# zxhuang1698/ShapeClipper

Hardware: AMD Instinct MI355X
Metric: train-step images/sec (Pix3D cfg, bs32/GPU) (higher is better)
Workload: dtype f32 (bf16x3-split MFMA, fp32 accumulate)

## Files before the change

### shapeclipper_amd/csrc/block.hip

```cpp
#include <hip/hip_runtime.h>
#include <stdint.h>

#include "shapeclipper_hip.h"


extern "C" int sc_basic_block_forward(const sc_block_args* a, void* stream) {
    if (!a || a->batch <= 0 || a->channels <= 0) return (int)hipErrorInvalidValue;
    const int B = a->batch, C = a->channels, hw = a->hw, HW = hw * hw, G = a->groups;
    auto conv = a->split ? sc_conv3x3_forward_split : sc_conv3x3_forward;
    int rc = conv(a->x, a->pf1, a->y1, a->conv_ws, B, C, C, hw, stream);
    if (rc) return rc;
    rc = sc_bn_act_forward(a->y1, nullptr, a->g1, a->b1, a->a1, a->st1, a->st1 + (size_t)G * C, a->rm1, a->rv1, a->nt1, a->bn_ws, B, C, HW, 1,
                           a->training, G, a->eps1, a->mom1, stream);
    if (rc) return rc;
    rc = conv(a->a1, a->pf2, a->y2, a->conv_ws, B, C, C, hw, stream);
    if (rc) return rc;
    return sc_bn_act_forward(a->y2, a->x, a->g2, a->b2, a->out, a->st2, a->st2 + (size_t)G * C, a->rm2, a->rv2, a->nt2, a->bn_ws, B, C, HW, 1,
                             a->training, G, a->eps2, a->mom2, stream);
}

extern "C" int sc_basic_block_backward(const sc_block_args* a, void* stream) {
    if (!a || a->batch <= 0 || a->channels <= 0 || !a->d_out) return (int)hipErrorInvalidValue;
    const int B = a->batch, C = a->channels, hw = a->hw, HW = hw * hw, G = a->groups;
    auto conv = a->split ? sc_conv3x3_forward_split : sc_conv3x3_forward;
    auto wgrad = a->split ? sc_conv3x3_wgrad_split : sc_conv3x3_wgrad;
    int rc = sc_bn_act_backward(a->d_out, a->y2, a->out, a->g2, a->b2, a->st2, a->st2 + (size_t)G * C, a->bn_ws, a->dy2, a->need_dx ? a->dres : nullptr,
                                a->dgb2, a->dgb2 + C, B, C, HW, 1, a->training, G, stream);
    if (rc) return rc;
    rc = conv(a->dy2, a->pb2, a->da1, a->conv_ws, B, C, C, hw, stream);
    if (rc) return rc;
    if (a->gw2) {
        rc = wgrad(a->dy2, a->a1, a->gw2, a->wgrad_ws, B, C, C, hw, stream);
        if (rc) return rc;
    }
    rc = sc_bn_act_backward(a->da1, a->y1, nullptr, a->g1, a->b1, a->st1, a->st1 + (size_t)G * C, a->bn_ws, a->dy1, nullptr, a->dgb1, a->dgb1 + C, B,
                            C, HW, 1, a->training, G, stream);
    if (rc) return rc;
    if (a->need_dx) {
        rc = sc_conv3x3_forward_add(a->dy1, a->pb1, a->dres, a->dx, a->conv_ws, B, C, C, hw, a->split, stream);
        if (rc) return rc;
    }
    if (a->gw1) rc = wgrad(a->dy1, a->x, a->gw1, a->wgrad_ws, B, C, C, hw, stream);
    return rc;
}
```

### shapeclipper_amd/csrc/conv3x3.hip

```cpp
#include <hip/hip_runtime.h>

#include <map>
#include <mutex>
#include <tuple>
#include <vector>

#include "grid_cus.hpp"
#include "shapeclipper_hip.h"

#ifndef SC_CONV_SPANS
#define SC_CONV_SPANS 1
#endif
#ifndef SC_CONV_ABLATE
#define SC_CONV_ABLATE 0
#endif

namespace sc {

#ifdef SC_CONV_PROFILE
__device__ unsigned long long* conv_prof_buf = nullptr;
#define CV_STAMP(ID) { const unsigned long long t_ = __builtin_amdgcn_s_memrealtime(); if (conv_prof_buf && tid == 0) conv_prof_buf[(size_t)g * 32 + (ID)] = t_; }
#else
#define CV_STAMP(ID)
#endif

typedef float f32x16 __attribute__((ext_vector_type(16)));
typedef __bf16 cv_bf16x8 __attribute__((ext_vector_type(8)));
typedef __bf16 cv_bf16x2 __attribute__((ext_vector_type(2)));
typedef __attribute__((address_space(3))) void* lptr_cv_t;

__device__ __forceinline__ void conv_glds16(const void* gsrc, unsigned lds_dst) {
// ... 395 lines not shown
        } else {
            float4* dst = reinterpret_cast<float4*>(partial + ((size_t)g * 2 + (item - sp.rounds)) * C::TILE);
#pragma unroll
            for (int i = 0; i < WM; ++i)
#pragma unroll
                for (int j = 0; j < WN; ++j)
#pragma unroll
                    for (int q = 0; q < 4; ++q) {
                        const float4 v = make_float4(acc[i][j][4 * q], acc[i][j][4 * q + 1], acc[i][j][4 * q + 2], acc[i][j][4 * q + 3]);
                        float4* d = dst + (((wave * WM + i) * WN + j) * 4 + q) * 64 + lane;
                        *d = v;
                    }
        }
#ifdef SC_CONV_PROFILE
        asm volatile("s_waitcnt vmcnt(0)" ::: "memory");
        CV_STAMP(sid + 3)
        if (conv_prof_buf && tid == 0) conv_prof_buf[(size_t)g * 32 + sid + 4] = (unsigned long long)(kb1 - kb0);
#endif
    }
    CV_STAMP(25)
}

template <class C>
__global__ __launch_bounds__(C::NT) void conv3x3_fixup_kernel(const float* __restrict__ partial, float* __restrict__ out, int batch,
                                                              int cin, int cout, int G, const int* __restrict__ spans,
                                                              const float* __restrict__ addend) {
    const int tid = threadIdx.x, lane = tid & 63, wave = tid >> 6;
    const int wm = wave / C::WGN, wn = wave % C::WGN;
    const int npix = batch * C::HWO, nct = (cout + C::CT - 1) / C::CT, tiles = ((npix + C::PT - 1) / C::PT) * nct * (C::BD2 ? 4 : 1);
    const int nk = conv_nk<C>(cin);
    const ConvSplit sp = conv_split(tiles, nk, G);
#ifdef SC_CONV_PROFILE
    if (conv_prof_buf && tid == 0) conv_prof_buf[(size_t)(8192 + blockIdx.x * 4 + blockIdx.y) * 2] = __builtin_amdgcn_s_memrealtime();
#endif
    const int t = blockIdx.x, r0 = 4 * blockIdx.y;
    const long long u0 = (long long)t * nk, u1 = u0 + nk;
    const int g_first = conv_span_owner(spans, sp, u0, G), g_last = conv_span_owner(spans, sp, u1 - 1, G);
    if (g_first == g_last && conv_span_at(spans, sp, g_first, nk) == u0 && conv_span_at(spans, sp, g_first + 1, nk) == u1) return;
    float acc[C::WM][C::WN][4];
#pragma unroll
    for (int i = 0; i < C::WM; ++i)
#pragma unroll
        for (int j = 0; j < C::WN; ++j)
#pragma unroll
            for (int r = 0; r < 4; ++r) acc[i][j][r] = 0.f;
    for (int g = g_first; g <= g_last; ++g) {
        const int which = (int)(conv_span_at(spans, sp, g, nk) / nk) == t ? 0 : 1;
        const float4* src = reinterpret_cast<const float4*>(partial + ((size_t)g * 2 + which) * C::TILE);
#pragma unroll
        for (int i = 0; i < C::WM; ++i)
#pragma unroll
            for (int j = 0; j < C::WN; ++j) {
                const float4 v = src[(((wave * C::WM + i) * C::WN + j) * 4 + (r0 >> 2)) * 64 + lane];
                acc[i][j][0] += v.x; acc[i][j][1] += v.y; acc[i][j][2] += v.z; acc[i][j][3] += v.w;
            }
    }
    const int tile = sp.rounds * G + t;
    int phase, pt, ct;
    conv_tile_decode<C>(tile, nct, phase, pt, ct);
#pragma unroll
    for (int j = 0; j < C::WN; ++j) {
        const int p = pt * C::PT + (wn * C::WN + j) * 32 + (lane & 31);
        if (p >= npix) continue;
        int cs;
        float* ob = conv_out_pixel<C>(out, p, phase, cout, cs);
#pragma unroll
        for (int i = 0; i < C::WM; ++i)
#pragma unroll
            for (int r = 0; r < 4; ++r) {
                const int co = ct * C::CT + (wm * C::WM + i) * 32 + r + 2 * r0 + 4 * (lane >> 5);
                if (co < cout) ob[(size_t)co * cs] = addend ? acc[i][j][r] + addend[(ob - out) + (size_t)co * cs] : acc[i][j][r];
            }
    }
#ifdef SC_CONV_PROFILE
    asm volatile("s_waitcnt vmcnt(0)" ::: "memory");
    if (conv_prof_buf && tid == 0) conv_prof_buf[(size_t)(8192 + blockIdx.x * 4 + blockIdx.y) * 2 + 1] = __builtin_amdgcn_s_memrealtime();
#endif
}

__device__ __forceinline__ float conv_w_at(const float* __restrict__ w, int cin, int cout, int co, int ci, int tap, int transpose_flip) {
    return transpose_flip ? w[((size_t)ci * cout + co) * 9 + (8 - tap)] : w[((size_t)co * cin + ci) * 9 + tap];
}
__device__ __forceinline__ unsigned conv_bf16_piece(float v, int pc) {
    const __bf16 h0 = (__bf16)v;
    const float r1 = v - (float)h0;
    const __bf16 h1 = (__bf16)r1;
    const __bf16 h2 = (__bf16)(r1 - (float)h1);
    const __bf16 h = pc == 0 ? h0 : pc == 1 ? h1 : h2;
    return (unsigned)__builtin_bit_cast(unsigned short, h);
}
__device__ __forceinline__ float conv_pack_word(const float* __restrict__ w, unsigned t, int CT, int nk, int cin, int cout, int flip,
                                                bool split) {
    if (!split) {
        const int s4 = (int)(t & 3);
        t >>= 2;
        const int cl = (int)(t % CT);
        t /= CT;
        const int h = (int)(t & 1);
        t >>= 1;
        const int tap = (int)(t % 9);
// ... 193 lines not shown
        U[G] = total;
        return pos >= total;
    };
    int lo = 2 * ((total + G - 1) / G), hi = lo + 4 * ov2 + 4;
    while (!build(hi)) hi += 2 * nk;
    while (lo < hi) {
        const int mid = (lo + hi) / 2;
        if (build(mid)) hi = mid; else lo = mid + 1;
    }
    (void)build(hi);
    SpanTable& t = cache[key];
    t.host = U;
    if (hipMalloc(&t.dev, (size_t)(G + 1) * sizeof(int)) != hipSuccess ||
        hipMemcpyAsync(t.dev, t.host.data(), (size_t)(G + 1) * sizeof(int), hipMemcpyHostToDevice, st) != hipSuccess ||
        hipStreamSynchronize(st) != hipSuccess) {
        (void)hipGetLastError();
        if (t.dev) (void)hipFree(t.dev);
        t.dev = nullptr;
    }
    return t.dev;
}

template <class C>
static int launch_conv(const float* x, const float* wpack, float* out, float* workspace, int batch, int cin, int cout, hipStream_t st,
                       const float* addend = nullptr) {
    if (cin % C::CB || batch <= 0) return (int)hipErrorInvalidValue;
    const int tiles = ((batch * C::HWO + C::PT - 1) / C::PT) * ((cout + C::CT - 1) / C::CT) * (C::BD2 ? 4 : 1), nk = conv_nk<C>(cin);
    const int G = conv_grid() * C::WGS_PER_CU;
    if (C::SPLIT && (long long)batch * cin * C::HW * 4 > 0x7fffffffLL) return (int)hipErrorInvalidValue;
    (void)hipFuncSetAttribute((const void*)conv3x3_kernel<C>, hipFuncAttributeMaxDynamicSharedMemorySize, C::LDS_BYTES);
    const ConvSplit sp = conv_split(tiles, nk, G);
    const int* spans = (SC_CONV_SPANS && sp.tail_tiles > 0 && sp.per_wg <= nk) ? conv_spans(sp.tail_tiles, nk, G, C::PT >= 512 ? 2 : 3, st) : nullptr;
    hipLaunchKernelGGL((conv3x3_kernel<C>), dim3(G), dim3(C::NT), C::LDS_BYTES, st, x, wpack, out, workspace, batch, cin, cout, spans, addend);
    if (sp.tail_tiles > 0)
        hipLaunchKernelGGL((conv3x3_fixup_kernel<C>), dim3(sp.tail_tiles, 4), dim3(C::NT), 0, st, workspace, out, batch, cin, cout, G, spans, addend);
    return (int)hipGetLastError();
}

}

extern "C" int sc_conv3x3_release_tables(void) {
    std::lock_guard<std::mutex> lock(sc::span_mu);
    int dev0 = 0;
    (void)hipGetDevice(&dev0);
    for (auto& kv : sc::span_cache)
        if (kv.second.dev) {
            (void)hipSetDevice(std::get<0>(kv.first));
            (void)hipFree(kv.second.dev);
        }
    sc::span_cache.clear();
    (void)hipSetDevice(dev0);
    return 0;
}

#define SC_CONV_DISPATCH(hw, CALL)                   \
    switch (hw) {                                    \
        case 56: return CALL(sc::Conv56);            \
        case 28: return CALL(sc::Conv28);            \
// ... 144 lines not shown
    }
    if (transpose_flip & 2) {
#define CALL(C) sc::launch_pack<C>(w, w_pack, cin, cout, transpose_flip & 1, (hipStream_t)stream)
        SC_CONV_DISPATCH_SPLIT(hw, CALL)
#undef CALL
    }
#define CALL(C) sc::launch_pack<C>(w, w_pack, cin, cout, transpose_flip & 1, (hipStream_t)stream)
    SC_CONV_DISPATCH(hw, CALL)
#undef CALL
}

extern "C" int sc_conv3x3_forward_add(const float* x, const float* w_pack, const float* addend, float* out, float* workspace, int batch, int cin,
                                      int cout, int hw, int split, void* stream) {
    if (split) {
#define CALL(C) sc::launch_conv<C>(x, w_pack, out, workspace, batch, cin, cout, (hipStream_t)stream, addend)
        SC_CONV_DISPATCH_SPLIT(hw, CALL)
#undef CALL
    }
#define CALL(C) sc::launch_conv<C>(x, w_pack, out, workspace, batch, cin, cout, (hipStream_t)stream, addend)
    SC_CONV_DISPATCH(hw, CALL)
#undef CALL
}

extern "C" int sc_conv3x3_forward(const float* x, const float* w_pack, float* out, float* workspace, int batch, int cin, int cout, int hw,
                                  void* stream) {
#define CALL(C) sc::launch_conv<C>(x, w_pack, out, workspace, batch, cin, cout, (hipStream_t)stream)
    SC_CONV_DISPATCH(hw, CALL)
#undef CALL
}
```

### shapeclipper_amd/csrc/conv3x3_wgrad.hip

```cpp
#include <hip/hip_runtime.h>

#include "grid_cus.hpp"
#include "shapeclipper_hip.h"

namespace sc {

typedef float wg_f32x16 __attribute__((ext_vector_type(16)));

#ifdef SC_WGRAD_PROFILE
__device__ unsigned long long* wgrad_prof_buf = nullptr;
#define WG_STAMP(ID) { const unsigned long long t_ = __builtin_amdgcn_s_memrealtime(); if (wgrad_prof_buf && tid == 0) wgrad_prof_buf[(size_t)blockIdx.x * 16 + (ID)] = t_; }
#define WG_ACCUM(ID, T0) { const unsigned long long t_ = __builtin_amdgcn_s_memrealtime(); if (wgrad_prof_buf && tid == 0) wgrad_prof_buf[(size_t)blockIdx.x * 16 + (ID)] += t_ - (T0); }
#else
#define WG_STAMP(ID)
#endif

template <int W_, int NR_, int NIMG_, int GS_, int S_ = 1>
struct WgCfg {
    static constexpr int W = W_, H = W_, NR = NR_, NIMG = NIMG_, GS = GS_, S = S_;
    static constexpr int HW = W * W;
    static constexpr int XW = S * W, XH = S * H, XHW = XW * XH;
    static constexpr int Wp = S == 1 ? W + 2 : XW + 1;
    static constexpr bool WHOLE = NR == H;
    static constexpr int SLOTW = (W + 2 * GS - 1) / (2 * GS) * (2 * GS);
    static constexpr int ROWS = NIMG * NR;
    static constexpr int NSLOT = ROWS * SLOTW;
    static constexpr int GST = NSLOT + (((NSLOT / GS) & 1) ? 0 : GS);
    static constexpr int PR = S == 1 ? NR + 2 : 2 * NR + 1;
    static constexpr int PATCH = NIMG * PR * Wp;
    static constexpr int LQ = (S == 1 ? PATCH : PATCH + 2 * GS + 2) | 1;
    static constexpr int LDS_FLOATS = 64 * GST + 64 * LQ > 4 * 48 * 64 ? 64 * GST + 64 * LQ : 4 * 48 * 64;
    static constexpr int CHUNK = W == 7 ? 49 : 56;
    static constexpr int RPC = CHUNK / W;
    static constexpr int XCHUNK = XW == 7 ? 49 : 56, XRPC = XCHUNK / XW;
    static constexpr int XROWS = WHOLE ? XH : PR;
    static constexpr int XCH = (XROWS + XRPC - 1) / XRPC, GCH = (NR + RPC - 1) / RPC;
    static constexpr int HR = ROWS / 2;
    static constexpr int GPR = SLOTW / (2 * GS);
    static constexpr int KH_A = HR * SLOTW;
    static constexpr int KH_B = NIMG == 2 ? PR * Wp : S * HR * Wp;
    static constexpr int NBV = S == 1 ? GS + 2 : 2 * GS + 1;
    static_assert(ROWS % 2 == 0 && H % NR == 0 && SLOTW % (2 * GS) == 0 && CHUNK % W == 0 && XCHUNK % XW == 0 && (S == 1 || S == 2), "K-step shape");
    static_assert(LDS_FLOATS * 4 <= 160 * 1024 && 4 * 48 * 64 <= LDS_FLOATS, "LDS");
};

template <class C>
__global__ __launch_bounds__(512, 1) void conv3x3_wgrad_kernel(const float* __restrict__ gy, const float* __restrict__ x,
                                                               float* __restrict__ partial, int batch, int cin, int cout, int S) {
    constexpr int W = C::W, H = C::H, HW = C::HW, Wp = C::Wp, GS = C::GS, NIMG = C::NIMG, NR = C::NR, ST = C::S;
    constexpr int XW = C::XW, XH = C::XH, XHW = C::XHW;
    extern __shared__ float4 wg_smem[];
    float* As = reinterpret_cast<float*>(wg_smem);
    float* Xs = As + 64 * C::GST;
    const int tid = threadIdx.x, lane = tid & 63, wave = __builtin_amdgcn_readfirstlane(tid >> 6), half = lane >> 5;
    const int wt = wave & 3, kh = wave >> 2;
    const int nti = cin / 64;
    const int blk = blockIdx.x / S, s = blockIdx.x - blk * S;
    const int co0 = (blk / nti) * 64, ci0 = (blk % nti) * 64;
    const int nimg_steps = NIMG == 2 ? (batch + 1) / 2 : batch * (H / NR);
    const int k_lo = (int)((long long)s * nimg_steps / S), k_hi = (int)((long long)(s + 1) * nimg_steps / S);

    for (int i = tid; i < C::LDS_FLOATS; i += 512) As[i] = 0.f;

    const bool lane_on = lane < C::CHUNK, xlane_on = lane < C::XCHUNK;
    const int lrow = lane / W, lx = lane - lrow * W;
    const int xlrow = lane / XW, xlx = lane - xlrow * XW;
    float xv[8][C::XCH * NIMG], gv[8][C::GCH * NIMG];
    auto load = [&](int kstep) {
        int b, y0;
        if (NIMG == 2) { b = 2 * kstep; y0 = 0; } else { b = kstep / (H / NR); y0 = (kstep - b * (H / NR)) * NR; }
#pragma unroll
        for (int im = 0; im < NIMG; ++im) {
            const bool img_ok = b + im < batch;
            const float* xb = x + ((size_t)(b + im) * cin + ci0 + 8 * wave) * XHW;
            const float* gb = gy + ((size_t)(b + im) * cout + co0 + 8 * wave) * HW;
#pragma unroll
            for (int c = 0; c < C::XCH; ++c) {
                const int yr = (C::WHOLE ? 0 : ST * y0 - 1) + c * C::XRPC + xlrow;
                const bool ok = xlane_on && img_ok && (unsigned)yr < (unsigned)XH && c * C::XRPC + xlrow < C::XROWS;
                const int off = yr * XW + xlx;
// ... 75 lines not shown
        }
        __syncthreads();
    }

    float* R = As;
#pragma unroll
    for (int pass = 0; pass < 3; ++pass) {
        if (kh == 1) {
#pragma unroll
            for (int t = 0; t < 3; ++t)
#pragma unroll
                for (int r = 0; r < 16; ++r) R[((wt * 3 + t) * 16 + r) * 64 + lane] = acc[pass * 3 + t][r];
        }
        __syncthreads();
        if (kh == 0) {
#pragma unroll
            for (int t = 0; t < 3; ++t)
#pragma unroll
                for (int r = 0; r < 16; ++r) acc[pass * 3 + t][r] += R[((wt * 3 + t) * 16 + r) * 64 + lane];
        }
        __syncthreads();
    }
    if (kh == 0) {
        float* dst = partial + (size_t)blockIdx.x * (64 * 64 * 9);
#pragma unroll
        for (int t = 0; t < 9; ++t)
#pragma unroll
            for (int r = 0; r < 16; ++r) dst[((wt * 9 + t) * 16 + r) * 64 + lane] = acc[t][r];
    }
}

__global__ __launch_bounds__(256) void conv3x3_wgrad_reduce_kernel(const float* __restrict__ partial, float* __restrict__ dw, int cin,
                                                                  int cout, int S) {
    __shared__ float part[4][64];
    const int nti = cin / 64, lane = threadIdx.x & 63, w = threadIdx.x >> 6;
    const int blk = blockIdx.x / 576, e = (blockIdx.x - blk * 576) * 64 + lane;
    const float* src = partial + (size_t)blk * S * 36864 + e;
    float s0 = 0.f, s1 = 0.f;
    int s = w;
    for (; s + 4 < S; s += 8) {
        s0 += src[(size_t)s * 36864];
        s1 += src[(size_t)(s + 4) * 36864];
    }
    if (s < S) s0 += src[(size_t)s * 36864];
    part[w][lane] = s0 + s1;
    __syncthreads();
    if (w == 0) {
        const float sum = (part[0][lane] + part[1][lane]) + (part[2][lane] + part[3][lane]);
        const int r = (e >> 6) & 15, t = (e >> 10) % 9, wt = e / (9 * 1024);
        const int co = (blk / nti) * 64 + (wt >> 1) * 32 + (r & 3) + 8 * (r >> 2) + 4 * (lane >> 5);
        const int ci = (blk % nti) * 64 + (wt & 1) * 32 + (lane & 31);
        dw[((size_t)co * cin + ci) * 9 + t] = sum;
    }
}

using Wg56 = WgCfg<56, 2, 1, 4>;
using Wg28 = WgCfg<28, 4, 1, 2>;
using Wg14 = WgCfg<14, 14, 1, 1>;
using Wg7 = WgCfg<7, 7, 2, 1>;
using Wg28S2 = WgCfg<28, 2, 1, 2, 2>;
using Wg14S2 = WgCfg<14, 2, 1, 1, 2>;
using Wg7S2 = WgCfg<7, 7, 2, 1, 2>;

typedef __bf16 wg_bf16x8 __attribute__((ext_vector_type(8)));
typedef float wg_f32x4 __attribute__((ext_vector_type(4)));
#ifndef SC_WGRAD_S16
#define SC_WGRAD_S16 0
#endif

template <int W_, int NR_, int NIMG_>
struct WsCfg {
    static constexpr int W = W_, H = W_, NR = NR_, NIMG = NIMG_, HW = W * W;
    static constexpr int SLOTS = W == 7 ? 8 : (W + 15) / 16 * 16;
    static constexpr int ROWS = NIMG * NR, NSLOT = ROWS * SLOTS, G = NSLOT / 16;
    static constexpr int ASTR = NSLOT + 8;
    static constexpr int Wp = SLOTS + 2, PR = NR + 2, PATCH = NIMG * PR * Wp;
    static constexpr int BSTR = (PATCH + 3) / 4 * 4 + 2;
    static constexpr bool WHOLE = NR == H;
    static constexpr int LDS_BYTES = 3 * 64 * (ASTR + BSTR) * 2;
    static constexpr int CHUNK = W == 7 ? 49 : 56, RPC = CHUNK / W;
    static constexpr int XROWS = WHOLE ? H : PR;
    static constexpr int XCH = (XROWS + RPC - 1) / RPC, GCH = (NR + RPC - 1) / RPC;
    static_assert(NSLOT % 16 == 0 && H % NR == 0 && LDS_BYTES <= 160 * 1024 && (W >= 14 || (NIMG == 2 && NR == 7)), "K-step shape");
    static constexpr int boff(int g, int h) {
        if (W == 7) { const int r = 2 * g + h; return ((r / 7) * PR + r % 7) * Wp; }
        const int r = g / (SLOTS / 16), gx = g % (SLOTS / 16);
        return ((r / NR) * PR + r % NR) * Wp + 16 * gx + 8 * h;
    }
};

template <class C>
__global__ __launch_bounds__(768, 1) void conv3x3_wgrad_split_kernel(const float* __restrict__ gy, const float* __restrict__ x,
                                                                     float* __restrict__ partial, int batch, int cin, int cout, int S) {
    constexpr int W = C::W, H = C::H, HW = C::HW, Wp = C::Wp, NIMG = C::NIMG, NR = C::NR;
    extern __shared__ float4 wg_smem[];
    __bf16* As = reinterpret_cast<__bf16*>(wg_smem);
    __bf16* Xs = As + 3 * 64 * C::ASTR;
    const int tid = threadIdx.x, lane = tid & 63, wave = __builtin_amdgcn_readfirstlane(tid >> 6), half = lane >> 5;
    const int wt = wave & 3, ky = wave >> 2;
    const int nti = cin / 64;
    const int blk = blockIdx.x / S, s = blockIdx.x - blk * S;
    const int co0 = (blk / nti) * 64, ci0 = (blk % nti) * 64;
    const int nimg_steps = NIMG == 2 ? (batch + 1) / 2 : batch * (H / NR);
    const int k_lo = (int)((long long)s * nimg_steps / S), k_hi = (int)((long long)(s + 1) * nimg_steps / S);

    for (int i = tid; i < C::LDS_BYTES / 16; i += 768) wg_smem[i] = make_float4(0.f, 0.f, 0.f, 0.f);

    const bool lane_on = lane < C::CHUNK, xrole = wave < 8;
    const int lrow = lane / W, lx = lane - lrow * W;
    constexpr int NSV = 8 * C::XCH * NIMG > 16 * C::GCH * NIMG ? 8 * C::XCH * NIMG : 16 * C::GCH * NIMG;
    float sv[NSV];
    auto load = [&](int kstep) {
        int b, y0;
        if (NIMG == 2) { b = 2 * kstep; y0 = 0; } else { b = kstep / (H / NR); y0 = (kstep - b * (H / NR)) * NR; }
        if (xrole) {
#pragma unroll
            for (int im = 0; im < NIMG; ++im) {
                const float* xb = x + ((size_t)(b + im) * cin + ci0 + 8 * wave) * HW;
#pragma unroll
                for (int c = 0; c < C::XCH; ++c) {
                    const int rr = c * C::RPC + lrow, yr = (C::WHOLE ? 0 : y0 - 1) + rr;
                    const bool ok = lane_on && b + im < batch && (unsigned)yr < (unsigned)H && rr < C::XROWS;
                    const int off = yr * W + lx;
#pragma unroll
// ... 143 lines not shown
#pragma unroll
                for (int q = 0; q < 5; ++q) d[pc][q] = Bb[pc * 32 * C::BSTR + bo + q];
            }
#pragma unroll
            for (int term = 0; term < 6; ++term) {
                constexpr int PA[6] = {0, 2, 1, 0, 1, 0}, PB[6] = {2, 0, 1, 1, 0, 0};
                const unsigned* q = d[PB[term]];
                const wg_bf16x8 av = __builtin_bit_cast(wg_bf16x8, a[PA[term]]);
                uint4 b0 = {q[0], q[1], q[2], q[3]}, b2 = {q[1], q[2], q[3], q[4]};
                uint4 b1 = {__builtin_amdgcn_alignbit(q[1], q[0], 16), __builtin_amdgcn_alignbit(q[2], q[1], 16),
                            __builtin_amdgcn_alignbit(q[3], q[2], 16), __builtin_amdgcn_alignbit(q[4], q[3], 16)};
                acc[0] = __builtin_amdgcn_mfma_f32_32x32x16_bf16(av, __builtin_bit_cast(wg_bf16x8, b0), acc[0], 0, 0, 0);
                acc[1] = __builtin_amdgcn_mfma_f32_32x32x16_bf16(av, __builtin_bit_cast(wg_bf16x8, b1), acc[1], 0, 0, 0);
                acc[2] = __builtin_amdgcn_mfma_f32_32x32x16_bf16(av, __builtin_bit_cast(wg_bf16x8, b2), acc[2], 0, 0, 0);
            }
        }
#endif
        __syncthreads();
#ifdef SC_WGRAD_PROFILE
        WG_ACCUM(5, ts1)
#endif
    }
    WG_STAMP(2)
    float* dst = partial + (size_t)blockIdx.x * (64 * 64 * 9);
#if SC_WGRAD_S16
#pragma unroll
    for (int t = 0; t < 3; ++t)
#pragma unroll
        for (int sa = 0; sa < 2; ++sa)
#pragma unroll
            for (int sb = 0; sb < 2; ++sb)
#pragma unroll
                for (int r = 0; r < 4; ++r)
                    dst[((wt * 9 + ky * 3 + t) * 16 + r + 4 * (2 * sa + (q4 >> 1))) * 64 + 16 * sb + l16 + 32 * (q4 & 1)] = acc[t][sa][sb][r];
#else
#pragma unroll
    for (int t = 0; t < 3; ++t)
#pragma unroll
        for (int r = 0; r < 16; ++r) dst[((wt * 9 + ky * 3 + t) * 16 + r) * 64 + lane] = acc[t][r];
#endif
#ifdef SC_WGRAD_PROFILE
    asm volatile("s_waitcnt vmcnt(0)" ::: "memory");
    WG_STAMP(3)
    if (wgrad_prof_buf && tid == 0) wgrad_prof_buf[(size_t)blockIdx.x * 16 + 6] = (unsigned long long)(k_hi - k_lo);
#endif
}

using Ws56 = WsCfg<56, 2, 1>;
using Ws28 = WsCfg<28, 4, 1>;
using Ws14 = WsCfg<14, 7, 1>;
using Ws7 = WsCfg<7, 7, 2>;

static int wg_cus() { return grid_cus(); }
static int wg_splits(int cin, int cout) {
    const int nblk = (cin / 64) * (cout / 64), s = wg_cus() / nblk;
    return s > 0 ? s : 1;
}

template <class C>
static int launch_wgrad(const float* gy, const float* x, float* dw, float* workspace, int batch, int cin, int cout, hipStream_t st) {
    if (cin % 64 || cout % 64 || batch <= 0) return (int)hipErrorInvalidValue;
    const int nblk = (cin / 64) * (cout / 64), S = wg_splits(cin, cout);
    (void)hipFuncSetAttribute((const void*)conv3x3_wgrad_kernel<C>, hipFuncAttributeMaxDynamicSharedMemorySize, C::LDS_FLOATS * 4);
    hipLaunchKernelGGL((conv3x3_wgrad_kernel<C>), dim3(nblk * S), dim3(512), C::LDS_FLOATS * 4, st, gy, x, workspace, batch, cin, cout, S);
    hipLaunchKernelGGL(conv3x3_wgrad_reduce_kernel, dim3(nblk * 576), dim3(256), 0, st, workspace, dw, cin, cout, S);
    return (int)hipGetLastError();
}

template <class C>
static int launch_wgrad_split(const float* gy, const float* x, float* dw, float* workspace, int batch, int cin, int cout, hipStream_t st) {
    if (cin % 64 || cout % 64 || batch <= 0) return (int)hipErrorInvalidValue;
    const int nblk = (cin / 64) * (cout / 64), S = wg_splits(cin, cout);
    (void)hipFuncSetAttribute((const void*)conv3x3_wgrad_split_kernel<C>, hipFuncAttributeMaxDynamicSharedMemorySize, C::LDS_BYTES);
    hipLaunchKernelGGL((conv3x3_wgrad_split_kernel<C>), dim3(nblk * S), dim3(768), C::LDS_BYTES, st, gy, x, workspace, batch, cin, cout, S);
    hipLaunchKernelGGL(conv3x3_wgrad_reduce_kernel, dim3(nblk * 576), dim3(256), 0, st, workspace, dw, cin, cout, S);
    return (int)hipGetLastError();
}

}

#ifdef SC_WGRAD_PROFILE
extern "C" int sc_wgrad_debug_set_prof(unsigned long long* buf) {
    return (int)hipMemcpyToSymbol(HIP_SYMBOL(sc::wgrad_prof_buf), &buf, sizeof(buf));
}
#endif
extern "C" int sc_conv3x3_wgrad_split(const float* gy, const float* x, float* dw, float* workspace, int batch, int cin, int cout, int hw, void* stream) {
    switch (hw) {
        case 56: return sc::launch_wgrad_split<sc::Ws56>(gy, x, dw, workspace, batch, cin, cout, (hipStream_t)stream);
        case 28: return sc::launch_wgrad_split<sc::Ws28>(gy, x, dw, workspace, batch, cin, cout, (hipStream_t)stream);
        case 14: return sc::launch_wgrad_split<sc::Ws14>(gy, x, dw, workspace, batch, cin, cout, (hipStream_t)stream);
        case 7: return sc::launch_wgrad_split<sc::Ws7>(gy, x, dw, workspace, batch, cin, cout, (hipStream_t)stream);
        default: return -1;
    }
}

extern "C" long long sc_conv3x3_wgrad_workspace_floats(int cin, int cout) {
    if (cin <= 0 || cout <= 0 || cin % 64 || cout % 64) return -1;
    return (long long)(cin / 64) * (cout / 64) * sc::wg_splits(cin, cout) * 36864;
}
// ... 20 lines not shown
```

### shapeclipper_amd/ops.py

```python
from __future__ import annotations

import collections
import ctypes
import weakref

import torch

from . import _lib
from .packing import n_tiles

_SCRATCH = {}


def _scratch(tag, dev, n_floats):
    if dev.type != "cuda":
        raise RuntimeError(_lib.NO_CPU)
    key = (tag, dev.index, torch._C._cuda_getCurrentRawStream(dev.index))
    buf = _SCRATCH.get(key)
    if buf is None or buf.numel() < n_floats:
        buf = _SCRATCH[key] = torch.empty(n_floats, device=dev, dtype=torch.float32)
    return buf


SDF_SCRATCH_FLOATS = 256 * 8 * 5 * 1024
# ... 979 lines not shown
def conv3x3_backward_weight(gy, x, split=False):
    lib = _lib.load()
    gy, x = _aligned(gy), _aligned(x)
    B, cout, H, _ = gy.shape
    cin = x.shape[1]
    n = lib.sc_conv3x3_wgrad_workspace_floats(cin, cout)
    if n < 0 or H not in CONV3X3_SIDES or x.shape[0] != B or tuple(x.shape[2:]) != (H, H):
        raise RuntimeError("shapeclipper_amd: sc_conv3x3_wgrad does not take gy %s with x %s" % (tuple(gy.shape), tuple(x.shape)))
    ws = _scratch("conv wgrad", x.device, n)
    dw = torch.empty(cout, cin, 3, 3, device=x.device, dtype=torch.float32)
    fn = lib.sc_conv3x3_wgrad_split if split else lib.sc_conv3x3_wgrad
    _lib.check(fn(_lib.ptr(gy), _lib.ptr(x), _lib.ptr(dw), _lib.ptr(ws), B, cin, cout, H, _lib.stream()), "sc_conv3x3_wgrad")
    return dw


class BlockArgs(ctypes.Structure):
    _fields_ = ([(n, ctypes.c_void_p) for n in ("x", "pf1", "pf2", "pb1", "pb2", "g1", "b1", "g2", "b2", "rm1", "rv1", "rm2", "rv2", "nt1", "nt2",
                                   "y1", "a1", "y2", "out", "st1", "st2", "conv_ws", "bn_ws", "wgrad_ws", "d_out",
                                   "dy2", "dres", "da1", "dy1", "dx", "gw1", "gw2", "dgb1", "dgb2")]
                + [(n, ctypes.c_int) for n in ("batch", "channels", "hw", "groups", "training", "split", "need_dx")]
                + [(n, ctypes.c_float) for n in ("mom1", "eps1", "mom2", "eps2")])


def _wgrad_workspace(x, cin, cout):
    return _scratch("conv wgrad", x.device, _lib.load().sc_conv3x3_wgrad_workspace_floats(cin, cout))


def basic_block_forward(x, pf1, pf2, g1, b1, g2, b2, bn1_state, bn2_state, split, groups):
    B, C, H, _ = x.shape
    rm1, rv1, nt1, training, mom1, eps1 = bn1_state
    rm2, rv2, nt2, _, mom2, eps2 = bn2_state
    y1, a1, y2, out = (torch.empty_like(x) for _ in range(4))
    st = torch.empty(2, 2, groups, C, device=x.device, dtype=torch.float32)
    a = BlockArgs()
    a.x, a.pf1, a.pf2 = x.data_ptr(), pf1.data_ptr(), pf2.data_ptr()
    a.g1, a.b1, a.g2, a.b2 = g1.data_ptr(), b1.data_ptr(), g2.data_ptr(), b2.data_ptr()
    a.rm1, a.rv1, a.nt1, a.rm2, a.rv2, a.nt2 = _p(rm1), _p(rv1), _p(nt1), _p(rm2), _p(rv2), _p(nt2)
    a.y1, a.a1, a.y2, a.out = y1.data_ptr(), a1.data_ptr(), y2.data_ptr(), out.data_ptr()
    a.st1, a.st2 = st[0].data_ptr(), st[1].data_ptr()
    a.conv_ws, a.bn_ws = _conv_workspace(x.device, H, split).data_ptr(), _bn_partial(x, groups)
    a.batch, a.channels, a.hw, a.groups, a.training, a.split = B, C, H, groups, 1 if training else 0, 1 if split else 0
    a.mom1, a.eps1, a.mom2, a.eps2 = mom1, eps1, mom2, eps2
    code = _lib.load().sc_basic_block_forward(ctypes.byref(a), _lib.raw_stream(x.get_device()))
    if code:
        _lib.check(code, "sc_basic_block_forward")
    return out, (y1, a1, y2, st[0], st[1])


def basic_block_backward(d_out, x, saved, out, pb1, pb2, g1, b1, g2, b2, training, split, groups, need_dx, need_w1, need_w2):
    y1, a1, y2, st1, st2 = saved
    B, C, H, _ = x.shape
    dy2, da1, dy1 = (torch.empty_like(x) for _ in range(3))
    dx, dres = (torch.empty_like(x), torch.empty_like(x)) if need_dx else (None, None)
    gw1 = torch.empty(C, C, 3, 3, device=x.device, dtype=torch.float32) if need_w1 else None
    gw2 = torch.empty(C, C, 3, 3, device=x.device, dtype=torch.float32) if need_w2 else None
    dgb = torch.empty(2, 2, C, device=x.device, dtype=torch.float32)
    a = BlockArgs()
    a.x, a.pb1, a.pb2, a.d_out = x.data_ptr(), pb1.data_ptr(), pb2.data_ptr(), d_out.data_ptr()
    a.g1, a.b1, a.g2, a.b2 = g1.data_ptr(), b1.data_ptr(), g2.data_ptr(), b2.data_ptr()
    a.y1, a.a1, a.y2, a.out, a.st1, a.st2 = y1.data_ptr(), a1.data_ptr(), y2.data_ptr(), out.data_ptr(), st1.data_ptr(), st2.data_ptr()
    a.dy2, a.da1, a.dy1, a.dres, a.dx = dy2.data_ptr(), da1.data_ptr(), dy1.data_ptr(), _p(dres), _p(dx)
    a.gw1, a.gw2, a.dgb1, a.dgb2 = _p(gw1), _p(gw2), dgb[0].data_ptr(), dgb[1].data_ptr()
    a.conv_ws, a.bn_ws = _conv_workspace(x.device, H, split).data_ptr(), _bn_partial(x, groups)
    a.wgrad_ws = _wgrad_workspace(x, C, C).data_ptr() if (need_w1 or need_w2) else None
    a.batch, a.channels, a.hw, a.groups, a.training, a.split, a.need_dx = B, C, H, groups, 1 if training else 0, 1 if split else 0, 1 if need_dx else 0
    code = _lib.load().sc_basic_block_backward(ctypes.byref(a), _lib.raw_stream(x.get_device()))
    if code:
        _lib.check(code, "sc_basic_block_backward")
    return dx, gw1, dgb[0, 0], dgb[0, 1], gw2, dgb[1, 0], dgb[1, 1]


def conv_stem_supported(x_shape, w_shape, stride=2, padding=3) -> bool:
    return (tuple(x_shape[1:]) == (3, 224, 224) and tuple(w_shape) == (64, 3, 7, 7) and stride in (2, (2, 2)) and padding in (3, (3, 3)))


def conv_stem_forward(x, w):
    lib = _lib.load()
    x, w = _aligned(x), _aligned(w)
    out = torch.empty(x.shape[0], 64, 112, 112, device=x.device, dtype=torch.float32)
    _lib.check(lib.sc_conv_stem_forward(_lib.ptr(x), _lib.ptr(w), _lib.ptr(out), x.shape[0], _lib.stream()), "sc_conv_stem_forward")
    return out


def conv_stem_backward_weight(gy, x):
    lib = _lib.load()
    gy, x = _aligned(gy), _aligned(x)
    ws = _scratch("conv stem", x.device, lib.sc_conv_stem_wgrad_workspace_floats())
# ... 552 lines not shown
```

Before: 999.0.

## Batch block-backward wgrads into one launch and fuse fixup with reductions

In the basic-block backward pass, the two weight-gradient convolutions now run as a single kernel launch whose grid covers both problems. Their split-K reductions are merged with the dx conv's tail-tile fixup into one combined finish kernel. This cuts the number of launches and lets the small reduce and fixup work share one grid, which should reduce tail underutilisation. In exchange it needs twice the wgrad workspace, and the wgrad for dy2 now runs after the dy1 BN backward instead of overlapping earlier in the stream order.

```diff
diff --git a/shapeclipper_amd/csrc/block.hip b/shapeclipper_amd/csrc/block.hip
--- a/shapeclipper_amd/csrc/block.hip
+++ b/shapeclipper_amd/csrc/block.hip
@@ -1,6 +1,7 @@
 #include <hip/hip_runtime.h>
 #include <stdint.h>
 
+#include "block_finish.hpp"
 #include "shapeclipper_hip.h"
 
 
@@ -22,24 +23,31 @@
 extern "C" int sc_basic_block_backward(const sc_block_args* a, void* stream) {
     if (!a || a->batch <= 0 || a->channels <= 0 || !a->d_out) return (int)hipErrorInvalidValue;
     const int B = a->batch, C = a->channels, hw = a->hw, HW = hw * hw, G = a->groups;
+    hipStream_t st = (hipStream_t)stream;
+    const long long per = sc_conv3x3_wgrad_workspace_floats(C, C);
+    if ((a->gw1 || a->gw2) && (per < 0 || !a->wgrad_ws)) return (int)hipErrorInvalidValue;
     auto conv = a->split ? sc_conv3x3_forward_split : sc_conv3x3_forward;
-    auto wgrad = a->split ? sc_conv3x3_wgrad_split : sc_conv3x3_wgrad;
     int rc = sc_bn_act_backward(a->d_out, a->y2, a->out, a->g2, a->b2, a->st2, a->st2 + (size_t)G * C, a->bn_ws, a->dy2, a->need_dx ? a->dres : nullptr,
                                 a->dgb2, a->dgb2 + C, B, C, HW, 1, a->training, G, stream);
     if (rc) return rc;
     rc = conv(a->dy2, a->pb2, a->da1, a->conv_ws, B, C, C, hw, stream);
     if (rc) return rc;
-    if (a->gw2) {
-        rc = wgrad(a->dy2, a->a1, a->gw2, a->wgrad_ws, B, C, C, hw, stream);
-        if (rc) return rc;
-    }
     rc = sc_bn_act_backward(a->da1, a->y1, nullptr, a->g1, a->b1, a->st1, a->st1 + (size_t)G * C, a->bn_ws, a->dy1, nullptr, a->dgb1, a->dgb1 + C, B,
                             C, HW, 1, a->training, G, stream);
     if (rc) return rc;
+    sc::ConvFixupJob fix;
     if (a->need_dx) {
-        rc = sc_conv3x3_forward_add(a->dy1, a->pb1, a->dres, a->dx, a->conv_ws, B, C, C, hw, a->split, stream);
+        rc = sc::conv3x3_forward_deferred(a->dy1, a->pb1, a->dres, a->dx, a->conv_ws, B, C, C, hw, a->split, st, &fix);
         if (rc) return rc;
     }
-    if (a->gw1) rc = wgrad(a->dy1, a->x, a->gw1, a->wgrad_ws, B, C, C, hw, stream);
-    return rc;
+    const float *gys[2], *xs[2];
+    sc::WgradReduceJob red[2];
+    int n = 0;
+    if (a->gw2) gys[n] = a->dy2, xs[n] = a->a1, red[n] = {a->wgrad_ws + (size_t)n * per, a->gw2}, ++n;
+    if (a->gw1) gys[n] = a->dy1, xs[n] = a->x, red[n] = {a->wgrad_ws + (size_t)n * per, a->gw1}, ++n;
+    if (n) {
+        rc = sc::conv3x3_wgrad_partials(gys, xs, n, a->wgrad_ws, B, C, C, hw, a->split, st);
+        if (rc) return rc;
+    }
+    return sc::conv_block_finish(fix, red, C, C, hw, a->split, st);
 }
diff --git a/shapeclipper_amd/csrc/block_finish.hpp b/shapeclipper_amd/csrc/block_finish.hpp
--- /dev/null
+++ b/shapeclipper_amd/csrc/block_finish.hpp
@@ -0,0 +1,27 @@
+#pragma once
+#include <hip/hip_runtime.h>
+
+namespace sc {
+
+struct ConvFixupJob {
+    const float* partial = nullptr;
+    float* out = nullptr;
+    const float* addend = nullptr;
+    const int* spans = nullptr;
+    int batch = 0, cin = 0, cout = 0, G = 0, tail_tiles = 0;
+};
+
+struct WgradReduceJob {
+    const float* partial = nullptr;
+    float* dw = nullptr;
+};
+
+int conv3x3_forward_deferred(const float* x, const float* w_pack, const float* addend, float* out, float* workspace, int batch, int cin,
+                             int cout, int hw, int split, hipStream_t st, ConvFixupJob* job);
+
+int conv3x3_wgrad_partials(const float* const* gy, const float* const* x, int n, float* workspace, int batch, int cin, int cout, int hw,
+                           int split, hipStream_t st);
+
+int conv_block_finish(const ConvFixupJob& fix, const WgradReduceJob (&red)[2], int cin, int cout, int hw, int split, hipStream_t st);
+
+}
diff --git a/shapeclipper_amd/csrc/conv3x3.hip b/shapeclipper_amd/csrc/conv3x3.hip
--- a/shapeclipper_amd/csrc/conv3x3.hip
+++ b/shapeclipper_amd/csrc/conv3x3.hip
@@ -5,8 +5,10 @@
 #include <tuple>
 #include <vector>
 
+#include "block_finish.hpp"
 #include "grid_cus.hpp"
 #include "shapeclipper_hip.h"
+#include "wgrad_reduce.hpp"
 
 #ifndef SC_CONV_SPANS
 #define SC_CONV_SPANS 1
@@ -448,21 +450,16 @@
 }
 
 template <class C>
-__global__ __launch_bounds__(C::NT) void conv3x3_fixup_kernel(const float* __restrict__ partial, float* __restrict__ out, int batch,
-                                                              int cin, int cout, int G, const int* __restrict__ spans,
-                                                              const float* __restrict__ addend) {
+__device__ __forceinline__ bool conv_fixup_body(const float* __restrict__ partial, float* __restrict__ out, int batch, int cin, int cout,
+                                                int G, const int* __restrict__ spans, const float* __restrict__ addend, int t, int r0) {
     const int tid = threadIdx.x, lane = tid & 63, wave = tid >> 6;
     const int wm = wave / C::WGN, wn = wave % C::WGN;
     const int npix = batch * C::HWO, nct = (cout + C::CT - 1) / C::CT, tiles = ((npix + C::PT - 1) / C::PT) * nct * (C::BD2 ? 4 : 1);
     const int nk = conv_nk<C>(cin);
     const ConvSplit sp = conv_split(tiles, nk, G);
-#ifdef SC_CONV_PROFILE
-    if (conv_prof_buf && tid == 0) conv_prof_buf[(size_t)(8192 + blockIdx.x * 4 + blockIdx.y) * 2] = __builtin_amdgcn_s_memrealtime();
-#endif
-    const int t = blockIdx.x, r0 = 4 * blockIdx.y;
     const long long u0 = (long long)t * nk, u1 = u0 + nk;
     const int g_first = conv_span_owner(spans, sp, u0, G), g_last = conv_span_owner(spans, sp, u1 - 1, G);
-    if (g_first == g_last && conv_span_at(spans, sp, g_first, nk) == u0 && conv_span_at(spans, sp, g_first + 1, nk) == u1) return;
+    if (g_first == g_last && conv_span_at(spans, sp, g_first, nk) == u0 && conv_span_at(spans, sp, g_first + 1, nk) == u1) return false;
     float acc[C::WM][C::WN][4];
 #pragma unroll
     for (int i = 0; i < C::WM; ++i)
@@ -498,10 +495,47 @@
                 if (co < cout) ob[(size_t)co * cs] = addend ? acc[i][j][r] + addend[(ob - out) + (size_t)co * cs] : acc[i][j][r];
             }
     }
+    return true;
+}
+
+template <class C>
+__global__ __launch_bounds__(C::NT) void conv3x3_fixup_kernel(const float* __restrict__ partial, float* __restrict__ out, int batch,
+                                                              int cin, int cout, int G, const int* __restrict__ spans,
+                                                              const float* __restrict__ addend) {
+#ifdef SC_CONV_PROFILE
+    const int tid = threadIdx.x;
+    if (conv_prof_buf && tid == 0) conv_prof_buf[(size_t)(8192 + blockIdx.x * 4 + blockIdx.y) * 2] = __builtin_amdgcn_s_memrealtime();
+#endif
+    if (!conv_fixup_body<C>(partial, out, batch, cin, cout, G, spans, addend, blockIdx.x, 4 * blockIdx.y)) return;
 #ifdef SC_CONV_PROFILE
     asm volatile("s_waitcnt vmcnt(0)" ::: "memory");
     if (conv_prof_buf && tid == 0) conv_prof_buf[(size_t)(8192 + blockIdx.x * 4 + blockIdx.y) * 2 + 1] = __builtin_amdgcn_s_memrealtime();
 #endif
+}
+
+struct BlockFinishArgs {
+    const float* partial;
+    float* out;
+    const float* addend;
+    const int* spans;
+    int batch, cin, cout, G, fix_blocks;
+    const float *rp0, *rp1;
+    float *dw0, *dw1;
+    int rcin, S, red_blocks;
+};
+
+template <class C>
+__global__ __launch_bounds__(C::NT) void conv_block_finish_kernel(const BlockFinishArgs a) {
+    static_assert(C::NT % 256 == 0 && 576 % (C::NT / 256) == 0, "whole reduction groups per workgroup");
+    __shared__ float part[C::NT / 64][64];
+    const int b = blockIdx.x;
+    if (b < a.fix_blocks) {
+        (void)conv_fixup_body<C>(a.partial, a.out, a.batch, a.cin, a.cout, a.G, a.spans, a.addend, b >> 2, 4 * (b & 3));
+        return;
+    }
+    const int rb = b - a.fix_blocks, second = rb >= a.red_blocks ? 1 : 0, q = threadIdx.x >> 8;
+    const int group = (rb - second * a.red_blocks) * (C::NT / 256) + q;
+    wgrad_reduce_group(second ? a.rp1 : a.rp0, second ? a.dw1 : a.dw0, a.rcin, a.S, group, threadIdx.x & 63, (threadIdx.x >> 6) & 3, part + 4 * q);
 }
 
 __device__ __forceinline__ float conv_w_at(const float* __restrict__ w, int cin, int cout, int co, int ci, int tap, int transpose_flip) {
@@ -741,8 +775,8 @@
 }
 
 template <class C>
-static int launch_conv(const float* x, const float* wpack, float* out, float* workspace, int batch, int cin, int cout, hipStream_t st,
-                       const float* addend = nullptr) {
+static int launch_conv_main(const float* x, const float* wpack, float* out, float* workspace, int batch, int cin, int cout, hipStream_t st,
+                            const float* addend, ConvFixupJob* job) {
     if (cin % C::CB || batch <= 0) return (int)hipErrorInvalidValue;
     const int tiles = ((batch * C::HWO + C::PT - 1) / C::PT) * ((cout + C::CT - 1) / C::CT) * (C::BD2 ? 4 : 1), nk = conv_nk<C>(cin);
     const int G = conv_grid() * C::WGS_PER_CU;
@@ -751,8 +785,44 @@
     const ConvSplit sp = conv_split(tiles, nk, G);
     const int* spans = (SC_CONV_SPANS && sp.tail_tiles > 0 && sp.per_wg <= nk) ? conv_spans(sp.tail_tiles, nk, G, C::PT >= 512 ? 2 : 3, st) : nullptr;
     hipLaunchKernelGGL((conv3x3_kernel<C>), dim3(G), dim3(C::NT), C::LDS_BYTES, st, x, wpack, out, workspace, batch, cin, cout, spans, addend);
-    if (sp.tail_tiles > 0)
-        hipLaunchKernelGGL((conv3x3_fixup_kernel<C>), dim3(sp.tail_tiles, 4), dim3(C::NT), 0, st, workspace, out, batch, cin, cout, G, spans, addend);
+    job->partial = workspace, job->out = out, job->addend = addend, job->spans = spans;
+    job->batch = batch, job->cin = cin, job->cout = cout, job->G = G, job->tail_tiles = sp.tail_tiles;
+    return (int)hipGetLastError();
+}
+
+template <class C>
+static int launch_conv(const float* x, const float* wpack, float* out, float* workspace, int batch, int cin, int cout, hipStream_t st,
+                       const float* addend = nullptr) {
+    ConvFixupJob f;
+    const int rc = launch_conv_main<C>(x, wpack, out, workspace, batch, cin, cout, st, addend, &f);
+    if (rc) return rc;
+    if (f.tail_tiles > 0)
+        hipLaunchKernelGGL((conv3x3_fixup_kernel<C>), dim3(f.tail_tiles, 4), dim3(C::NT), 0, st, f.partial, f.out, f.batch, f.cin, f.cout, f.G, f.spans,
+                           f.addend);
+    return (int)hipGetLastError();
+}
+
+template <class C>
+static int launch_block_finish(const ConvFixupJob& fix, const WgradReduceJob (&red)[2], int cin, int cout, hipStream_t st) {
+    BlockFinishArgs a{};
+    if (fix.tail_tiles > 0) {
+        a.partial = fix.partial, a.out = fix.out, a.addend = fix.addend, a.spans = fix.spans;
+        a.batch = fix.batch, a.cin = fix.cin, a.cout = fix.cout, a.G = fix.G, a.fix_blocks = 4 * fix.tail_tiles;
+    }
+    int nred = 0;
+    for (const WgradReduceJob& r : red)
+        if (r.dw) {
+            (nred ? a.rp1 : a.rp0) = r.partial;
+            (nred ? a.dw1 : a.dw0) = r.dw;
+            ++nred;
+        }
+    if (nred) {
+        if (cin <= 0 || cout <= 0 || cin % 64 || cout % 64) return (int)hipErrorInvalidValue;
+        a.rcin = cin, a.S = wg_splits(cin, cout), a.red_blocks = (cin / 64) * (cout / 64) * 576 / (C::NT / 256);
+    }
+    const int blocks = a.fix_blocks + nred * a.red_blocks;
+    if (blocks == 0) return 0;
+    hipLaunchKernelGGL((conv_block_finish_kernel<C>), dim3(blocks), dim3(C::NT), 0, st, a);
     return (int)hipGetLastError();
 }
 
@@ -943,6 +1013,25 @@
 #undef CALL
 }
 
+int sc::conv3x3_forward_deferred(const float* x, const float* w_pack, const float* addend, float* out, float* workspace, int batch, int cin,
+                                 int cout, int hw, int split, hipStream_t st, ConvFixupJob* job) {
+#define CALL(C) sc::launch_conv_main<C>(x, w_pack, out, workspace, batch, cin, cout, st, addend, job)
+    if (split) {
+        SC_CONV_DISPATCH_SPLIT(hw, CALL)
+    }
+    SC_CONV_DISPATCH(hw, CALL)
+#undef CALL
+}
+
+int sc::conv_block_finish(const ConvFixupJob& fix, const WgradReduceJob (&red)[2], int cin, int cout, int hw, int split, hipStream_t st) {
+#define CALL(C) sc::launch_block_finish<C>(fix, red, cin, cout, st)
+    if (split) {
+        SC_CONV_DISPATCH_SPLIT(hw, CALL)
+    }
+    SC_CONV_DISPATCH(hw, CALL)
+#undef CALL
+}
+
 extern "C" int sc_conv3x3_forward(const float* x, const float* w_pack, float* out, float* workspace, int batch, int cin, int cout, int hw,
                                   void* stream) {
 #define CALL(C) sc::launch_conv<C>(x, w_pack, out, workspace, batch, cin, cout, (hipStream_t)stream)
diff --git a/shapeclipper_amd/csrc/conv3x3_wgrad.hip b/shapeclipper_amd/csrc/conv3x3_wgrad.hip
--- a/shapeclipper_amd/csrc/conv3x3_wgrad.hip
+++ b/shapeclipper_amd/csrc/conv3x3_wgrad.hip
@@ -1,9 +1,18 @@
 #include <hip/hip_runtime.h>
 
+#include "block_finish.hpp"
 #include "grid_cus.hpp"
 #include "shapeclipper_hip.h"
+#include "wgrad_reduce.hpp"
 
 namespace sc {
+
+struct WgradProblems {
+    const float *gy0, *x0;
+    float* partial0;
+    const float *gy1, *x1;
+    float* partial1;
+};
 
 typedef float wg_f32x16 __attribute__((ext_vector_type(16)));
 
@@ -45,8 +54,7 @@
 };
 
 template <class C>
-__global__ __launch_bounds__(512, 1) void conv3x3_wgrad_kernel(const float* __restrict__ gy, const float* __restrict__ x,
-                                                               float* __restrict__ partial, int batch, int cin, int cout, int S) {
+__global__ __launch_bounds__(512, 1) void conv3x3_wgrad_kernel(const WgradProblems pr, int batch, int cin, int cout, int S) {
     constexpr int W = C::W, H = C::H, HW = C::HW, Wp = C::Wp, GS = C::GS, NIMG = C::NIMG, NR = C::NR, ST = C::S;
     constexpr int XW = C::XW, XH = C::XH, XHW = C::XHW;
     extern __shared__ float4 wg_smem[];
@@ -55,7 +63,11 @@
     const int tid = threadIdx.x, lane = tid & 63, wave = __builtin_amdgcn_readfirstlane(tid >> 6), half = lane >> 5;
     const int wt = wave & 3, kh = wave >> 2;
     const int nti = cin / 64;
-    const int blk = blockIdx.x / S, s = blockIdx.x - blk * S;
+    const int per = nti * (cout / 64) * S, prob = (int)blockIdx.x >= per ? 1 : 0, bid = (int)blockIdx.x - prob * per;
+    const float* __restrict__ gy = prob ? pr.gy1 : pr.gy0;
+    const float* __restrict__ x = prob ? pr.x1 : pr.x0;
+    float* __restrict__ partial = prob ? pr.partial1 : pr.partial0;
+    const int blk = bid / S, s = bid - blk * S;
     const int co0 = (blk / nti) * 64, ci0 = (blk % nti) * 64;
     const int nimg_steps = NIMG == 2 ? (batch + 1) / 2 : batch * (H / NR);
     const int k_lo = (int)((long long)s * nimg_steps / S), k_hi = (int)((long long)(s + 1) * nimg_steps / S);
@@ -177,7 +189,7 @@
         __syncthreads();
     }
     if (kh == 0) {
-        float* dst = partial + (size_t)blockIdx.x * (64 * 64 * 9);
+        float* dst = partial + (size_t)bid * (64 * 64 * 9);
 #pragma unroll
         for (int t = 0; t < 9; ++t)
 #pragma unroll
@@ -188,25 +200,8 @@
 __global__ __launch_bounds__(256) void conv3x3_wgrad_reduce_kernel(const float* __restrict__ partial, float* __restrict__ dw, int cin,
                                                                   int cout, int S) {
     __shared__ float part[4][64];
-    const int nti = cin / 64, lane = threadIdx.x & 63, w = threadIdx.x >> 6;
-    const int blk = blockIdx.x / 576, e = (blockIdx.x - blk * 576) * 64 + lane;
-    const float* src = partial + (size_t)blk * S * 36864 + e;
-    float s0 = 0.f, s1 = 0.f;
-    int s = w;
-    for (; s + 4 < S; s += 8) {
-        s0 += src[(size_t)s * 36864];
-        s1 += src[(size_t)(s + 4) * 36864];
-    }
-    if (s < S) s0 += src[(size_t)s * 36864];
-    part[w][lane] = s0 + s1;
-    __syncthreads();
-    if (w == 0) {
-        const float sum = (part[0][lane] + part[1][lane]) + (part[2][lane] + part[3][lane]);
-        const int r = (e >> 6) & 15, t = (e >> 10) % 9, wt = e / (9 * 1024);
-        const int co = (blk / nti) * 64 + (wt >> 1) * 32 + (r & 3) + 8 * (r >> 2) + 4 * (lane >> 5);
-        const int ci = (blk % nti) * 64 + (wt & 1) * 32 + (lane & 31);
-        dw[((size_t)co * cin + ci) * 9 + t] = sum;
-    }
+    (void)cout;
+    wgrad_reduce_group(partial, dw, cin, S, blockIdx.x, threadIdx.x & 63, threadIdx.x >> 6, part);
 }
 
 using Wg56 = WgCfg<56, 2, 1, 4>;
@@ -245,8 +240,7 @@
 };
 
 template <class C>
-__global__ __launch_bounds__(768, 1) void conv3x3_wgrad_split_kernel(const float* __restrict__ gy, const float* __restrict__ x,
-                                                                     float* __restrict__ partial, int batch, int cin, int cout, int S) {
+__global__ __launch_bounds__(768, 1) void conv3x3_wgrad_split_kernel(const WgradProblems pr, int batch, int cin, int cout, int S) {
     constexpr int W = C::W, H = C::H, HW = C::HW, Wp = C::Wp, NIMG = C::NIMG, NR = C::NR;
     extern __shared__ float4 wg_smem[];
     __bf16* As = reinterpret_cast<__bf16*>(wg_smem);
@@ -254,7 +248,11 @@
     const int tid = threadIdx.x, lane = tid & 63, wave = __builtin_amdgcn_readfirstlane(tid >> 6), half = lane >> 5;
     const int wt = wave & 3, ky = wave >> 2;
     const int nti = cin / 64;
-    const int blk = blockIdx.x / S, s = blockIdx.x - blk * S;
+    const int per = nti * (cout / 64) * S, prob = (int)blockIdx.x >= per ? 1 : 0, bid = (int)blockIdx.x - prob * per;
+    const float* __restrict__ gy = prob ? pr.gy1 : pr.gy0;
+    const float* __restrict__ x = prob ? pr.x1 : pr.x0;
+    float* __restrict__ partial = prob ? pr.partial1 : pr.partial0;
+    const int blk = bid / S, s = bid - blk * S;
     const int co0 = (blk / nti) * 64, ci0 = (blk % nti) * 64;
     const int nimg_steps = NIMG == 2 ? (batch + 1) / 2 : batch * (H / NR);
     const int k_lo = (int)((long long)s * nimg_steps / S), k_hi = (int)((long long)(s + 1) * nimg_steps / S);
@@ -444,7 +442,7 @@
 #endif
     }
     WG_STAMP(2)
-    float* dst = partial + (size_t)blockIdx.x * (64 * 64 * 9);
+    float* dst = partial + (size_t)bid * (64 * 64 * 9);
 #if SC_WGRAD_S16
 #pragma unroll
     for (int t = 0; t < 3; ++t)
@@ -473,30 +471,62 @@
 using Ws14 = WsCfg<14, 7, 1>;
 using Ws7 = WsCfg<7, 7, 2>;
 
-static int wg_cus() { return grid_cus(); }
-static int wg_splits(int cin, int cout) {
-    const int nblk = (cin / 64) * (cout / 64), s = wg_cus() / nblk;
-    return s > 0 ? s : 1;
+template <class C>
+static int launch_wgrad_partials(const WgradProblems& pr, int n, int batch, int cin, int cout, hipStream_t st) {
+    if (cin % 64 || cout % 64 || batch <= 0 || n < 1 || n > 2) return (int)hipErrorInvalidValue;
+    const int nblk = (cin / 64) * (cout / 64), S = wg_splits(cin, cout);
+    (void)hipFuncSetAttribute((const void*)conv3x3_wgrad_kernel<C>, hipFuncAttributeMaxDynamicSharedMemorySize, C::LDS_FLOATS * 4);
+    hipLaunchKernelGGL((conv3x3_wgrad_kernel<C>), dim3(n * nblk * S), dim3(512), C::LDS_FLOATS * 4, st, pr, batch, cin, cout, S);
+    return (int)hipGetLastError();
+}
+
+template <class C>
+static int launch_wgrad_split_partials(const WgradProblems& pr, int n, int batch, int cin, int cout, hipStream_t st) {
+    if (cin % 64 || cout % 64 || batch <= 0 || n < 1 || n > 2) return (int)hipErrorInvalidValue;
+    const int nblk = (cin / 64) * (cout / 64), S = wg_splits(cin, cout);
+    (void)hipFuncSetAttribute((const void*)conv3x3_wgrad_split_kernel<C>, hipFuncAttributeMaxDynamicSharedMemorySize, C::LDS_BYTES);
+    hipLaunchKernelGGL((conv3x3_wgrad_split_kernel<C>), dim3(n * nblk * S), dim3(768), C::LDS_BYTES, st, pr, batch, cin, cout, S);
+    return (int)hipGetLastError();
+}
+
+static int launch_wgrad_reduce(const float* workspace, float* dw, int cin, int cout, hipStream_t st) {
+    hipLaunchKernelGGL(conv3x3_wgrad_reduce_kernel, dim3((cin / 64) * (cout / 64) * 576), dim3(256), 0, st, workspace, dw, cin, cout, wg_splits(cin, cout));
+    return (int)hipGetLastError();
 }
 
 template <class C>
 static int launch_wgrad(const float* gy, const float* x, float* dw, float* workspace, int batch, int cin, int cout, hipStream_t st) {
-    if (cin % 64 || cout % 64 || batch <= 0) return (int)hipErrorInvalidValue;
-    const int nblk = (cin / 64) * (cout / 64), S = wg_splits(cin, cout);
-    (void)hipFuncSetAttribute((const void*)conv3x3_wgrad_kernel<C>, hipFuncAttributeMaxDynamicSharedMemorySize, C::LDS_FLOATS * 4);
-    hipLaunchKernelGGL((conv3x3_wgrad_kernel<C>), dim3(nblk * S), dim3(512), C::LDS_FLOATS * 4, st, gy, x, workspace, batch, cin, cout, S);
-    hipLaunchKernelGGL(conv3x3_wgrad_reduce_kernel, dim3(nblk * 576), dim3(256), 0, st, workspace, dw, cin, cout, S);
-    return (int)hipGetLastError();
+    const int rc = launch_wgrad_partials<C>(WgradProblems{gy, x, workspace, nullptr, nullptr, nullptr}, 1, batch, cin, cout, st);
+    return rc ? rc : launch_wgrad_reduce(workspace, dw, cin, cout, st);
 }
 
 template <class C>
 static int launch_wgrad_split(const float* gy, const float* x, float* dw, float* workspace, int batch, int cin, int cout, hipStream_t st) {
-    if (cin % 64 || cout % 64 || batch <= 0) return (int)hipErrorInvalidValue;
-    const int nblk = (cin / 64) * (cout / 64), S = wg_splits(cin, cout);
-    (void)hipFuncSetAttribute((const void*)conv3x3_wgrad_split_kernel<C>, hipFuncAttributeMaxDynamicSharedMemorySize, C::LDS_BYTES);
-    hipLaunchKernelGGL((conv3x3_wgrad_split_kernel<C>), dim3(nblk * S), dim3(768), C::LDS_BYTES, st, gy, x, workspace, batch, cin, cout, S);
-    hipLaunchKernelGGL(conv3x3_wgrad_reduce_kernel, dim3(nblk * 576), dim3(256), 0, st, workspace, dw, cin, cout, S);
-    return (int)hipGetLastError();
+    const int rc = launch_wgrad_split_partials<C>(WgradProblems{gy, x, workspace, nullptr, nullptr, nullptr}, 1, batch, cin, cout, st);
+    return rc ? rc : launch_wgrad_reduce(workspace, dw, cin, cout, st);
+}
+
+int conv3x3_wgrad_partials(const float* const* gy, const float* const* x, int n, float* workspace, int batch, int cin, int cout, int hw, int split,
+                           hipStream_t st) {
+    if (n < 1 || n > 2 || cin <= 0 || cout <= 0 || cin % 64 || cout % 64) return (int)hipErrorInvalidValue;
+    const size_t per = (size_t)(cin / 64) * (cout / 64) * wg_splits(cin, cout) * 36864;
+    const WgradProblems pr{gy[0], x[0], workspace, n > 1 ? gy[1] : nullptr, n > 1 ? x[1] : nullptr, n > 1 ? workspace + per : nullptr};
+    if (split) {
+        switch (hw) {
+            case 56: return launch_wgrad_split_partials<Ws56>(pr, n, batch, cin, cout, st);
+            case 28: return launch_wgrad_split_partials<Ws28>(pr, n, batch, cin, cout, st);
+            case 14: return launch_wgrad_split_partials<Ws14>(pr, n, batch, cin, cout, st);
+            case 7: return launch_wgrad_split_partials<Ws7>(pr, n, batch, cin, cout, st);
+            default: return -1;
+        }
+    }
+    switch (hw) {
+        case 56: return launch_wgrad_partials<Wg56>(pr, n, batch, cin, cout, st);
+        case 28: return launch_wgrad_partials<Wg28>(pr, n, batch, cin, cout, st);
+        case 14: return launch_wgrad_partials<Wg14>(pr, n, batch, cin, cout, st);
+        case 7: return launch_wgrad_partials<Wg7>(pr, n, batch, cin, cout, st);
+        default: return -1;
+    }
 }
 
 }
diff --git a/shapeclipper_amd/csrc/wgrad_reduce.hpp b/shapeclipper_amd/csrc/wgrad_reduce.hpp
--- /dev/null
+++ b/shapeclipper_amd/csrc/wgrad_reduce.hpp
@@ -0,0 +1,36 @@
+#pragma once
+#include <hip/hip_runtime.h>
+
+#include "grid_cus.hpp"
+
+namespace sc {
+
+inline int wg_splits(int cin, int cout) {
+    const int nblk = (cin / 64) * (cout / 64), s = grid_cus() / nblk;
+    return s > 0 ? s : 1;
+}
+
+__device__ __forceinline__ void wgrad_reduce_group(const float* __restrict__ partial, float* __restrict__ dw, int cin, int S, int group,
+                                                   int lane, int w, float (*part)[64]) {
+    const int nti = cin / 64;
+    const int blk = group / 576, e = (group - blk * 576) * 64 + lane;
+    const float* src = partial + (size_t)blk * S * 36864 + e;
+    float s0 = 0.f, s1 = 0.f;
+    int s = w;
+    for (; s + 4 < S; s += 8) {
+        s0 += src[(size_t)s * 36864];
+        s1 += src[(size_t)(s + 4) * 36864];
+    }
+    if (s < S) s0 += src[(size_t)s * 36864];
+    part[w][lane] = s0 + s1;
+    __syncthreads();
+    if (w == 0) {
+        const float sum = (part[0][lane] + part[1][lane]) + (part[2][lane] + part[3][lane]);
+        const int r = (e >> 6) & 15, t = (e >> 10) % 9, wt = e / (9 * 1024);
+        const int co = (blk / nti) * 64 + (wt >> 1) * 32 + (r & 3) + 8 * (r >> 2) + 4 * (lane >> 5);
+        const int ci = (blk % nti) * 64 + (wt & 1) * 32 + (lane & 31);
+        dw[((size_t)co * cin + ci) * 9 + t] = sum;
+    }
+}
+
+}
diff --git a/shapeclipper_amd/ops.py b/shapeclipper_amd/ops.py
--- a/shapeclipper_amd/ops.py
+++ b/shapeclipper_amd/ops.py
@@ -1025,8 +1025,8 @@
                 + [(n, ctypes.c_float) for n in ("mom1", "eps1", "mom2", "eps2")])
 
 
-def _wgrad_workspace(x, cin, cout):
-    return _scratch("conv wgrad", x.device, _lib.load().sc_conv3x3_wgrad_workspace_floats(cin, cout))
+def _wgrad_workspace(x, cin, cout, problems=1):
+    return _scratch("conv wgrad", x.device, problems * _lib.load().sc_conv3x3_wgrad_workspace_floats(cin, cout))
 
 
 def basic_block_forward(x, pf1, pf2, g1, b1, g2, b2, bn1_state, bn2_state, split, groups):
@@ -1065,7 +1065,7 @@
     a.dy2, a.da1, a.dy1, a.dres, a.dx = dy2.data_ptr(), da1.data_ptr(), dy1.data_ptr(), _p(dres), _p(dx)
     a.gw1, a.gw2, a.dgb1, a.dgb2 = _p(gw1), _p(gw2), dgb[0].data_ptr(), dgb[1].data_ptr()
     a.conv_ws, a.bn_ws = _conv_workspace(x.device, H, split).data_ptr(), _bn_partial(x, groups)
-    a.wgrad_ws = _wgrad_workspace(x, C, C).data_ptr() if (need_w1 or need_w2) else None
+    a.wgrad_ws = _wgrad_workspace(x, C, C, int(need_w1) + int(need_w2)).data_ptr() if (need_w1 or need_w2) else None
     a.batch, a.channels, a.hw, a.groups, a.training, a.split, a.need_dx = B, C, H, groups, 1 if training else 0, 1 if split else 0, 1 if need_dx else 0
     code = _lib.load().sc_basic_block_backward(ctypes.byref(a), _lib.raw_stream(x.get_device()))
     if code:
```

Result: no change. 989.6 (-0.9%).
